# brownvc/gftorf

Measured on AMD Instinct MI355X. Metric: train iters/sec (fwd+bwd raster) + Mpix/s, 1M Gaussians @ 640x480 ToF, higher is better.
Workload: dtype f32; 1 GPU; 1M Gaussians, 640x480, SH deg 3, RGB+ToF phasor, forward+backward; P=1000000, W=640, H=480, sh_degree=3, P_visible=954168, num_rendered=3638471, longest_tile_list=0

## Files before the change

gftorf_amd/_lib.py:

```python
import ctypes as C
import os

_HERE = os.path.dirname(os.path.abspath(__file__))
LIB_PATH = os.path.join(_HERE, "libgftorf_rast.so")
ABI_VERSION = 15
DEFORM_MAX_INPUTS = 96
ACC_STRIDE = 16

_lib = None

_fp = C.c_void_p


class Config(C.Structure):
    _fields_ = [
        ("P", C.c_int32), ("D", C.c_int32), ("M", C.c_int32), ("M_p", C.c_int32),
        ("W", C.c_int32), ("H", C.c_int32),
        ("tanfovx", C.c_float), ("tanfovy", C.c_float), ("scale_modifier", C.c_float),
        ("near_n", C.c_float), ("far_n", C.c_float), ("depth_range", C.c_float),
        ("phase_offset", C.c_float), ("dc_offset", C.c_float),
        ("use_view_dependent_phase", C.c_int32), ("prefiltered", C.c_int32), ("debug", C.c_int32),
        ("want_backward", C.c_int32),
        ("acc_zeroed", C.c_int32),
        ("grads_zeroed", C.c_int32),
# ... 89 lines not shown

class DeformParams(C.Structure):
    _fields_ = [("linear_w", _fp * 8), ("linear_b", _fp * 8), ("xyz_w", _fp), ("xyz_b", _fp), ("r_w", _fp), ("r_b", _fp),
                ("g_w", _fp), ("g_b", _fp), ("b_w", _fp), ("b_b", _fp)]


DEFORM_FIELDS = [f[0] for f in DeformParams._fields_]


class AdamTensor(C.Structure):
    _fields_ = [("param", _fp), ("grad", _fp), ("exp_avg", _fp), ("exp_avg_sq", _fp), ("n", C.c_int64), ("lr", C.c_double),
                ("step", C.c_int64)]

EXPORTS = [
    "gft_abi_version", "gft_lazy_sort", "gft_last_error", "gft_geom_bytes", "gft_image_bytes", "gft_cell_sched_words", "gft_binning_bytes", "gft_acc_bytes",
    "gft_det_partials_bytes", "gft_get_layout", "gft_binning_capacity", "gft_set_binning_mode", "gft_binning_mode", "gft_set_render_mode", "gft_forward_preprocess", "gft_forward_render", "gft_forward", "gft_forward_enqueue", "gft_backward", "gft_grads_rezero",
    "gft_mark_visible", "gft_profile_enable", "gft_profile_reset", "gft_profile_read",
    "gft_assemble_scratch_bytes", "gft_assemble_forward", "gft_assemble_num_dynamic", "gft_assemble_backward",
    "gft_knn_scratch_bytes", "gft_knn_mean_dist2", "gft_adam_step", "gft_adam_step_multi", "gft_adam_step_rows", "gft_adam_step_multi_dev",
    "gft_deform_inputs", "gft_deform_packed_bytes", "gft_deform_saved_bytes", "gft_deform_scratch_bytes", "gft_deform_pack",
    "gft_deform_forward", "gft_deform_backward", "gft_deform_compact", "gft_deform_rows_work_bytes", "gft_deform_backward_rows",
    "gft_ssim_blocks", "gft_ssim_l2_forward", "gft_ssim_l2_backward",
    "gft_image_loss_forward", "gft_image_loss_backward", "gft_pixel_loss_blocks", "gft_pixel_loss_forward", "gft_pixel_loss_backward",
    "gft_densify_stats", "gft_rows_rank_scratch_bytes", "gft_rows_rank", "gft_rows_rank_dev", "gft_rows_gather", "gft_rows_any_nonzero",
]
FLOW_EXPORTS = ["gft_flow_loss_blocks", "gft_flow_loss_forward", "gft_flow_loss_backward", "gft_flow_points", "gft_flow_project",
                "gft_flow_project_backward"]
FEATURE_EXPORTS = ["gft_render_features", "gft_render_features_backward"]


def load():
# ... 16 lines not shown
    lib.gft_image_bytes.argtypes = [C.c_int32, C.c_int32]
    lib.gft_cell_sched_words.restype = C.c_size_t
    lib.gft_cell_sched_words.argtypes = [C.c_int32, C.c_int32]
    lib.gft_binning_bytes.restype = C.c_size_t
    lib.gft_binning_bytes.argtypes = [C.c_int64, C.c_int32, C.c_int32]
    lib.gft_acc_bytes.restype = C.c_size_t
    lib.gft_acc_bytes.argtypes = [C.c_int32]
    lib.gft_det_partials_bytes.restype = C.c_size_t
    lib.gft_det_partials_bytes.argtypes = [C.c_int64, C.c_int32, C.c_int32]
    lib.gft_binning_capacity.restype = C.c_int64
    lib.gft_binning_capacity.argtypes = [C.c_size_t, C.c_int32, C.c_int32]
    lib.gft_set_binning_mode.restype = C.c_int
    lib.gft_set_binning_mode.argtypes = [C.c_int]
    lib.gft_set_render_mode.restype = C.c_int
    lib.gft_set_render_mode.argtypes = [C.c_int]
    lib.gft_binning_mode.restype = C.c_int
    lib.gft_binning_mode.argtypes = [C.POINTER(Config)]
    lib.gft_get_layout.restype = C.c_int
    lib.gft_get_layout.argtypes = [C.c_int32, C.c_int32, C.c_int32, C.c_int64, C.POINTER(Layout)]
    lib.gft_forward_preprocess.restype = C.c_int
    lib.gft_forward_preprocess.argtypes = [C.c_void_p, C.POINTER(Config), C.POINTER(ForwardIO),
                                           C.POINTER(C.c_int64), C.POINTER(C.c_int64)]
    lib.gft_forward_render.restype = C.c_int
    lib.gft_adam_step.restype = C.c_int
    lib.gft_adam_step.argtypes = [C.c_void_p, C.c_int64, C.c_void_p, C.c_void_p, C.c_void_p, C.c_void_p,
                                  C.c_double, C.c_double, C.c_double, C.c_double, C.c_double, C.c_int64]
    lib.gft_adam_step_multi.restype = C.c_int
    lib.gft_adam_step_multi.argtypes = [C.c_void_p, C.c_int32, C.POINTER(AdamTensor), C.c_double, C.c_double, C.c_double,
                                        C.c_double]
    lib.gft_adam_step_multi_dev.restype = C.c_int
# ... 173 lines not shown
```

gftorf_amd/csrc/gft_api.hip:

```cpp
#include "gft_internal.h"

#include <stdarg.h>
#include <stdio.h>
#include <string.h>
#include <cstdlib>
#include <mutex>
#include <vector>

static thread_local char g_err[512] = "";

int gft_fail(const char* fmt, ...)
{
    va_list ap;
    va_start(ap, fmt);
    vsnprintf(g_err, sizeof(g_err), fmt, ap);
    va_end(ap);
    return 1;
}

extern "C" const char* gft_last_error(void) { return g_err; }
extern "C" int gft_abi_version(void) { return GFT_ABI_VERSION; }
static size_t point_list_slots(int64_t binning_instances, int32_t W, int32_t H)
{
    if (binning_instances <= 0) return 0;
// ... 29 lines not shown
    L->geom_need = o;     o = align_up(o + p);
    L->geom_blockhist = o; o = align_up(o + ((p + BIN_CHUNK - 1) / BIN_CHUNK) * GFT_BLOCKHIST_TILES * 2);
    L->geom_total = o;

    const size_t n = (size_t)W * (size_t)H;
    const size_t T = (size_t)((W + GFT_TILE_X - 1) / GFT_TILE_X) * (size_t)((H + GFT_TILE_Y - 1) / GFT_TILE_Y);
    o = 0;
    L->img_pix_state = o;   o = align_up(o + n * 16);
    L->img_ranges = o;      o = align_up(o + T * 8);
    L->img_tile_max = o;    o = align_up(o + T * 4 * 4);
    L->img_ctrl = o;        o += (GFT_CTRL_WORDS + GFT_TICKET_WORDS) * 4;
    L->img_tile_cnt = o;    o += T * 4;
    L->img_tile_cut = o;    o += T * 4;
    L->img_super_tab = o;   o = align_up(o + 4 * (size_t)GFT_SUPER_CELLS * 4);
    L->img_tile_cursor = o; o = align_up(o + T * 4);
    L->img_tile_order = o;  o = align_up(o + T * 4);
    L->img_front_len = o;   o = align_up(o + T * 4);
    L->img_unit_flag = o;   o = align_up(o + T * 16);
    L->img_resume_state = o; o = align_up(o + n * 64);
    L->img_pix_sums = o;    o = align_up(o + n * 32);
    L->img_snaps = o;       o = align_up(o + 4 * T * (size_t)(gft_bwd_segments(T) - 1) * GFT_SNAP_F4 * 64 * 16);
    L->img_total = o;

    const size_t r = (size_t)(R > 0 ? R : 0);
    o = 0;
    L->bin_keys = o;        o = align_up(o + r * 8);
    L->bin_point_list = o;  o = align_up(o + (r ? T * (size_t)GFT_HEAD_SLOT + r : 0) * 4);
    L->bin_total = o + GFT_ALIGN;
}

GeomView gft_geom_view(void* base, const gft_layout& L)
// ... 13 lines not shown
}

ImgView gft_img_view(void* base, const gft_layout& L)
{
    char* b = (char*)base;
    ImgView v;
    v.pix_state = (float4*)(b + L.img_pix_state);
    v.ranges = (uint2*)(b + L.img_ranges);
    v.tile_max = (uint32_t*)(b + L.img_tile_max);
    v.ctrl = (uint32_t*)(b + L.img_ctrl);
    v.tile_cnt = (uint32_t*)(b + L.img_tile_cnt);
    v.tile_cut = (uint32_t*)(b + L.img_tile_cut);
    v.super_tab = (uint32_t*)(b + L.img_super_tab);
    v.tile_cursor = (uint32_t*)(b + L.img_tile_cursor);
    v.tile_order = (uint32_t*)(b + L.img_tile_order);
    v.front_len = (uint32_t*)(b + L.img_front_len);
    v.unit_flag = (uint32_t*)(b + L.img_unit_flag);
    v.resume_state = (float4*)(b + L.img_resume_state);
    v.pix_sums = (float4*)(b + L.img_pix_sums);
    v.snaps = (float4*)(b + L.img_snaps);
    return v;
}

BinView gft_bin_view(void* base, const gft_layout& L)
{
    char* b = (char*)base;
    BinView v;
    v.keys = (uint64_t*)(b + L.bin_keys);
    v.point_list = (uint32_t*)(b + L.bin_point_list);
    return v;
// ... 294 lines not shown
    if (m < 0) {
        const char* e = getenv("GFT_LAZY_BIN");
        m = e ? (atoi(e) != 0) : 1;
        g_binning_mode.store(m);
    }
    return m != 0 && lazy_sort_enabled() && gft_tile_pull_ok(*cfg);
}
extern "C" int gft_binning_mode(const gft_config* cfg) { return (cfg && pull_enabled(cfg)) ? 1 : 0; }

static std::atomic<int> g_render_mode{-2};
extern "C" int gft_set_render_mode(int mode)
{
    g_render_mode.store(mode < 0 ? -2 : (mode ? 1 : 0));
    return 0;
}
int gft_render_mode()
{
    int m = g_render_mode.load();
    if (m == -2) {
        const char* e = getenv("GFT_FWD_SEG");
        m = e ? (atoi(e) != 0 ? 1 : 0) : -1;
        g_render_mode.store(m);
    }
    return m;
}

static int enqueue_count(hipStream_t s, const gft_config* cfg, const gft_forward_io* io, const GeomView& g, const ImgView& im,
                         uint32_t* mail_dev, uint32_t seq, bool pull, int64_t status_cap = -1);

static int enqueue_stage1(hipStream_t s, const gft_config* cfg, const gft_forward_io* io, const GeomView& g,
// ... 131 lines not shown
    if (binning_instances < 0 || binning_instances > 0xffffffffll) return gft_fail("gft_forward_render: bad instance count");
    if (binning_instances > 0 && !io->binning) return gft_fail("gft_forward_render: binning buffer is NULL");
    if (cfg->P > 0 && (!io->geom || !io->radii || !io->pixels)) return gft_fail("gft_forward_render: geom/radii/pixels NULL");
    hipStream_t s = (hipStream_t)hip_stream;
    const int64_t R = cfg->P == 0 ? 0 : binning_instances;
    gft_layout L;
    gft_compute_layout(cfg->P, cfg->W, cfg->H, R, &L);
    GeomView g = gft_geom_view(io->geom, L);
    ImgView im = gft_img_view(io->img, L);
    BinView b = gft_bin_view(io->binning, L);
    const bool pull = cfg->P > 0 && pull_enabled(cfg);
    if (cfg->P == 0 || (pull && R == 0)) {
        const int gx = (cfg->W + GFT_TILE_X - 1) / GFT_TILE_X, gy = (cfg->H + GFT_TILE_Y - 1) / GFT_TILE_Y;
        GFT_CHECK_HIP(gft_zero_async(im.ranges, (size_t)gx * gy * sizeof(uint2), s));
        if (cfg->P == 0) GFT_CHECK_HIP(gft_zero_async(im.ctrl, GFT_CTRL_WORDS * sizeof(uint32_t), s));
    }
    return enqueue_stage2(s, cfg, io, g, im, b, R > 0, max_tile_list, cfg->P > 0, (uint32_t)R, pull, io->tile_hints != nullptr);
}

extern "C" int gft_forward(void* hip_stream, const gft_config* cfg, const gft_forward_io* io,
                           const gft_forward_hints* hints, gft_forward_report* report)
{
    if (report) memset(report, 0, sizeof(*report));
    if (check_config(cfg)) return 1;
    if (!io || !hints || !report) return gft_fail("gft_forward: NULL argument");
    if (check_stage2(io, "gft_forward")) return 1;
    const int64_t binning_instances = hints->binning_instances;
    if (binning_instances < 0 || binning_instances > 0xffffffffll) return gft_fail("gft_forward: bad instance count");
    if (cfg->P == 0) return gft_forward_render(hip_stream, cfg, io, 0, 0);
    if (check_stage1(cfg, io, "gft_forward")) return 1;
// ... 170 lines not shown
```

gftorf_amd/csrc/gft_appearance.h:

```cpp
#pragma once
#include "gft_internal.h"

#pragma clang fp contract(off)

struct PreFwdArgs {
    gft_config c;
    gft_forward_io io;
    GeomView g;
    uint32_t* ctrl;
    uint32_t clear_words;
    uint32_t* mail;
    int defer_appearance;
    float focal_x, focal_y, dist2phase;
    int gx, gy;
    int stage_sh, stage_shp;
    const uint32_t* prev_w;
    uint32_t* fwd_order;
    int T;
};

inline PreFwdArgs gft_pre_fwd_args(const gft_config& c, const gft_forward_io& io, const GeomView& g, const ImgView& im,
                                   uint32_t* mail, bool defer_appearance)
{
    PreFwdArgs a;
    a.c = c;
    a.io = io;
    a.g = g;
    a.ctrl = im.ctrl;
    a.mail = mail;
    a.defer_appearance = defer_appearance ? 1 : 0;
    {
        const size_t T = (size_t)((c.W + GFT_TILE_X - 1) / GFT_TILE_X) * (size_t)((c.H + GFT_TILE_Y - 1) / GFT_TILE_Y);
        a.clear_words = (uint32_t)(GFT_CTRL_WORDS + GFT_TICKET_WORDS + 2 * T + GFT_SUPER_CELLS);
    }
    a.focal_y = c.H / (2.0f * c.tanfovy);
    a.focal_x = c.W / (2.0f * c.tanfovx);
    a.dist2phase = 4.0f * 3.14159265358979323846f / c.depth_range;
    a.gx = (c.W + GFT_TILE_X - 1) / GFT_TILE_X;
    a.gy = (c.H + GFT_TILE_Y - 1) / GFT_TILE_Y;
    a.stage_sh = a.stage_shp = 0;
    a.prev_w = nullptr; a.fwd_order = nullptr; a.T = a.gx * a.gy;
    return a;
}
// ... 347 lines not shown
```

gftorf_amd/csrc/gft_internal.h:

```cpp
#pragma once
#include <hip/hip_runtime.h>
#include <stdint.h>
#include <stddef.h>
#include "gftorf_rast.h"

#include <atomic>
#include <cstdlib>

#define GFT_ALIGN 256

inline hipError_t gft_lds_opt_in(const void* kernel, size_t bytes, std::atomic<uint64_t>& done)
{
    int dev = 0;
    hipError_t e = hipGetDevice(&dev);
    if (e != hipSuccess) return e;
    const uint64_t bit = dev >= 0 && dev < 64 ? 1ull << dev : 0ull;
    if (bit && (done.load(std::memory_order_acquire) & bit)) return hipSuccess;
    e = hipFuncSetAttribute(kernel, hipFuncAttributeMaxDynamicSharedMemorySize, (int)bytes);
    if (e == hipSuccess && bit) done.fetch_or(bit, std::memory_order_release);
    return e;
}
#define GFT_BLOCK 256
#define GFT_NUM_ACC 15

// ... 9 lines not shown
    uint16_t* blockhist;
};

struct ImgView {
    float4* pix_state;
    float4* pix_sums;
    float4* snaps;
    uint2* ranges;
    uint32_t* tile_max;
    uint32_t* ctrl;
    uint32_t* tile_cnt;
    uint32_t* tile_cut;
    uint32_t* super_tab;
    uint32_t* tile_cursor;
    uint32_t* tile_order;
    uint32_t* front_len;
    uint32_t* unit_flag;
    float4* resume_state;
};

struct BinView {
    uint64_t* keys;
    uint32_t* point_list;
};

#define GFT_CTRL_TOTAL 0
#define GFT_CTRL_FLAGS 1
#define GFT_CTRL_MAXCNT 2
#define GFT_CTRL_NFLAG 4
#define GFT_CTRL_DONE 3
// ... 4 lines not shown
#define GFT_CTRL_NHINT 8
#define GFT_CTRL_RSUM 9
#define GFT_CTRL_FWDORDER 10
#define GFT_CTRL_ORDER_OK 11
#define GFT_CTRL_WORDS 16
__device__ __forceinline__ void gft_status_sticky(uint32_t* mail, uint32_t post, uint32_t R)
{
    if (!post) return;
    mail[GFT_STATUS_CAP] = post - 1u;
    if (R > post - 1u) {
        __hip_atomic_fetch_add(&mail[GFT_STATUS_OVERFLOWS], 1u, __ATOMIC_RELAXED, __HIP_MEMORY_SCOPE_SYSTEM);
        __hip_atomic_fetch_max(&mail[GFT_STATUS_MAX_R], R, __ATOMIC_RELAXED, __HIP_MEMORY_SCOPE_SYSTEM);
    }
}
#define GFT_TICKET_WORDS 32
#define GFT_SUPER_MAX 1024
#define GFT_SLAB_MAX 16
#define GFT_SUPER_CELLS (GFT_SUPER_MAX * GFT_SLAB_MAX)
#define GFT_DEPTH_BINS 4096
#define GFT_HEAD_SLOT 2048u
#define GFT_HEAD_DIRECT 2048u
#define GFT_HEAD_TARGET 940u
#define GFT_NO_TAIL 0xffffffffu
#define GFT_BLOCKHIST_TILES 2048
#ifndef BIN_THREADS
#define BIN_THREADS 1024
#endif
#ifndef BIN_ITEMS
#define BIN_ITEMS 4
#endif
// ... 249 lines not shown
```

gftorf_amd/csrc/gft_render_walk.h:

```cpp
#pragma once
#include "gft_internal.h"

struct RenderFwdArgs {
    int W, H, gx, T;
    const uint2* __restrict__ ranges;
    const uint32_t* __restrict__ point_list;
    const float4* __restrict__ rec_a;
    const float4* __restrict__ rec_b;
    const float* __restrict__ bg;
    int64_t bsc, bsy, bsx;
    float dc_offset;
    const float* dc_offset_dev;
    float4* __restrict__ pix_state;
    float4* __restrict__ pix_sums;
    uint32_t* __restrict__ quad_max;
    float* out_color; float* out_phasor; float* out_depth; float* out_normal; float* out_acc;
    float* out_entropy; float* out_dd; float* out_ad; float* out_distribution;
    float* pixels;
    const uint32_t* __restrict__ ctrl;
    uint32_t cap;
    const uint32_t* __restrict__ tile_cut;
    float4* __restrict__ snaps;
    int nsnap;
    const uint32_t* __restrict__ front_len;
    uint32_t* __restrict__ unit_flag;
    uint32_t* nflag;
    float4* __restrict__ resume_state;
    int resume;
    uint8_t* __restrict__ hint_out;
    const uint32_t* __restrict__ fwd_order;
    const uint32_t* __restrict__ fwd_order_ok;
    uint32_t* __restrict__ weights_out;
};

RenderFwdArgs gft_render_fwd_args(const gft_config& c, const gft_forward_io& io, const GeomView& g, const ImgView& im,
                                  const BinView& b, bool check_cap, uint32_t cap, int lazy, bool pull);

namespace {

#define RB 64

__device__ __forceinline__ float gft_exp(float x) { return __builtin_amdgcn_exp2f(x * 1.4426950408889634f); }

__device__ __forceinline__ unsigned long long wave_ballot(bool p) { return __builtin_amdgcn_ballot_w64(p); }

__device__ __forceinline__ float sel_mask(unsigned long long m, float a, float b)
{
// ... 235 lines not shown
```

gftorf_amd/csrc/k_preprocess.hip:

```cpp
#include "gft_internal.h"
#include "gft_appearance.h"
#include <mutex>

#pragma clang fp contract(off)

namespace {

template <int NC>
__device__ __forceinline__ void sh_backward(int deg, int M, float x, float y, float z, const float* sh,
                                            const float* dres, float* dsh, float* ddir)
{
    float ddx[NC], ddy[NC], ddz[NC];
#pragma unroll
    for (int c = 0; c < NC; c++) {
        ddx[c] = 0.f; ddy[c] = 0.f; ddz[c] = 0.f;
        dsh[c] = SH_C0 * dres[c];
    }
    int written = 1;
    if (deg > 0) {
        const float d1 = -SH_C1 * y, d2 = SH_C1 * z, d3 = -SH_C1 * x;
#pragma unroll
        for (int c = 0; c < NC; c++) {
            const float s1 = sh[1 * NC + c], s2 = sh[2 * NC + c], s3 = sh[3 * NC + c];
            ddx[c] = -SH_C1 * s3;
// ... 234 lines not shown
                    store_rec_a(a, idx, sg, vx, vy, vz);
                    if (!a.defer_appearance) appearance_fwd(a, idx, lane, sh_l, shp_l, px, py, pz, vx, vy, vz, phase_offset);
                    radius = (int)sg.my_radius;
                    tiles = area;
                    rect = make_ushort4((unsigned short)x0, (unsigned short)y0, (unsigned short)x1, (unsigned short)y1);
                }
            }
        }
        a.io.radii[idx] = radius;
        a.io.pixels[idx] = 0.0f;
        a.g.tiles[idx] = tiles;
        a.g.rect[idx] = rect;
        a.g.need[idx] = 0;
    }
    for (uint32_t w = (uint32_t)idx; w < a.clear_words; w += gridDim.x * PRE_BLOCK) a.ctrl[w] = 0u;
}

#define APP_THREADS 256
#define APP_CHUNK_OF(words) ((words) * 4 * APP_THREADS)
template <int WORDS>
__global__ __launch_bounds__(APP_THREADS) void k_appearance(PreFwdArgs a, uint32_t cap)
{
    constexpr int APP_CHUNK = APP_CHUNK_OF(WORDS);
    __shared__ uint32_t s_ids[APP_CHUNK];
    __shared__ uint32_t s_n;
    if (a.ctrl[GFT_CTRL_TOTAL] > cap) return;
    const float phase_offset = gft_offset_value(a.io.phase_offset_dev, a.c.phase_offset);
    const int tid = threadIdx.x, lane = tid & 63;
    if (blockIdx.x == 0 && a.prev_w != nullptr && a.prev_w[4 * a.T] == 1u) {
        gft_tile_order_block(a.T, a.prev_w, a.fwd_order);
// ... 722 lines not shown
```

gftorf_amd/csrc/k_render.hip:

```cpp
#include "gft_internal.h"
#include "gft_render_walk.h"

namespace {

typedef unsigned int u32x2 __attribute__((ext_vector_type(2)));

__device__ __forceinline__ int unit_of_block(int b, int V)
{
    const int chunk = (V + 7) >> 3;
    return (b & 7) * chunk + (b >> 3);
}

__global__ __launch_bounds__(64) void k_render_fwd(RenderFwdArgs a)
{
    __shared__ float4 sA[RB * 2];
    __shared__ float4 sB[RB * 2];

    const float dc_offset = gft_offset_value(a.dc_offset_dev, a.dc_offset);
    if (a.ctrl && a.ctrl[GFT_CTRL_TOTAL] > a.cap) return;
    if (a.resume && *a.nflag == 0u) return;
    const int V = a.T * 4;
    int v;
    if (a.fwd_order && *a.fwd_order_ok) {
        const int xcd = (int)blockIdx.x & 7, qslot = (int)blockIdx.x >> 3;
        const int rank = 8 * (qslot >> 2) + xcd;
        if (rank >= a.T) return;
        v = (int)a.fwd_order[rank] * 4 + (qslot & 3);
    } else {
        if (((int)blockIdx.x >> 3) >= ((V + 7) >> 3)) return;
        v = unit_of_block(blockIdx.x, V);
    }
    if (v >= V) return;
    render_fwd_walk(a, v, (int)threadIdx.x, sA, sB, dc_offset);
}

#define FSEG_WAVES_MAX 8
#define FSEG_MIN_LEN 128
#define FSEG_SPEC_MAX 512

template <int FSEG_WAVES>
__global__ __launch_bounds__(64 * FSEG_WAVES) __attribute__((amdgpu_waves_per_eu(7, 7))) void k_render_fwd_seg(RenderFwdArgs a)
{
    __shared__ float4 sStage[FSEG_WAVES][RB * 4];
    __shared__ float sT[FSEG_WAVES][64];
    __shared__ uint8_t sCnt[FSEG_WAVES][FSEG_SPEC_MAX];

    const float dc_offset = gft_offset_value(a.dc_offset_dev, a.dc_offset);
    if (a.ctrl && a.ctrl[GFT_CTRL_TOTAL] > a.cap) return;
// ... 401 lines not shown
    int split;
    int nseg;
    const float4* __restrict__ snaps;
    const uint32_t* __restrict__ front_len;
    const uint32_t* __restrict__ quad_max;
    const uint32_t* __restrict__ order;
    const uint32_t* __restrict__ order_ok;
    const uint32_t* __restrict__ order_fwd;
    const uint32_t* __restrict__ order_fwd_ok;
    const float* __restrict__ g_color; const float* __restrict__ g_phasor; const float* __restrict__ g_depth;
    const float* __restrict__ g_acc; const float* __restrict__ g_dd;
    const uint32_t* __restrict__ ctrl;
    uint32_t cap;
    float* acc;
    float* det;
};

__device__ __forceinline__ float swap32_add(float x, float y)
{
    const u32x2 r = __builtin_amdgcn_permlane32_swap(__float_as_uint(x), __float_as_uint(y), false, false);
    return __uint_as_float(r.x) + __uint_as_float(r.y);
}

__device__ __forceinline__ float swap16_add(float x, float y)
{
    const u32x2 r = __builtin_amdgcn_permlane16_swap(__float_as_uint(x), __float_as_uint(y), false, false);
    return __uint_as_float(r.x) + __uint_as_float(r.y);
}

__device__ __forceinline__ float row_fold4(float t0, float t1, float t2, float t3)
// ... 39 lines not shown

__device__ __forceinline__ float wave_reduce16(v2f L01, v2f L23, v2f L45, v2f L67, v2f H01, v2f H23, v2f H45, v2f H67)
{
    const v2f s01 = swap32_add2(L01, H01), s23 = swap32_add2(L23, H23);
    const v2f s45 = swap32_add2(L45, H45), s67 = swap32_add2(L67, H67);
    const v2f t01 = swap16_add2(s01, s45), t23 = swap16_add2(s23, s67);
    return row_fold4(t01.x, t01.y, t23.x, t23.y);
}

__global__ __launch_bounds__(1024) void k_tile_order(int T, const uint32_t* __restrict__ quad_max,
                                                     uint32_t* __restrict__ order)
{
    gft_tile_order_block(T, quad_max, order);
}

__global__ __launch_bounds__(64) void k_render_bwd(RenderBwdArgs a)
{
    __shared__ float4 sA[RB * 2];
    __shared__ float4 sB[RB * 2];
    __shared__ uint32_t sId[RB];

    if (a.ctrl[GFT_CTRL_TOTAL] > a.cap) return;
    const float dc_offset = gft_offset_value(a.dc_offset_dev, a.dc_offset);
    const int per_seg = (int)gridDim.x / a.nseg;
    const int sgroup = (int)blockIdx.x / per_seg;
    const int bid = (int)blockIdx.x - sgroup * per_seg;
    const int xcd = bid & 7, qslot = bid >> 3;
    const int rank = 8 * (qslot >> 2) + xcd;
    if (rank >= a.T) return;
    const uint32_t* order = a.order;
    bool ordered = order && (a.order_ok == nullptr || *a.order_ok != 0u);
    if (order && a.order_fwd && *a.order_fwd_ok != 0u) { order = a.order_fwd; ordered = true; }
    const int v_unit = (int)(ordered ? order[rank] : (uint32_t)rank) * 4 + (qslot & 3);
    const int tmax = (int)a.quad_max[v_unit];
    if (tmax == 0) return;
    int ncut = 0;
    if (a.split) {
        const int head = a.front_len ? (int)a.front_len[v_unit >> 2] : tmax;
        const int lim = min(tmax, head);
        ncut = lim > 0 ? (lim - 1) / GFT_SEG_LEN : 0;
        if (ncut > a.nseg - 1) ncut = a.nseg - 1;
    }
    const bool front_first = a.T > GFT_FWD_ORDER_MAX_TILES && ncut >= 1 && tmax - ncut * GFT_SEG_LEN <= GFT_SEG_LEN;
    int seg;
    if (sgroup == 0) seg = front_first ? 0 : ncut;
    else if (sgroup == 1) { if (ncut < 1) return; seg = front_first ? ncut : 0; }
    else { seg = sgroup - 1; if (seg >= ncut) return; }
    const int lo_last = seg * GFT_SEG_LEN;
    const int hi_first = seg == ncut ? tmax : lo_last + GFT_SEG_LEN;
    const int tile = v_unit >> 2, quad = v_unit & 3;
    const int lane = threadIdx.x;
    const int tx = tile % a.gx, ty = tile / a.gx;
    const int qx0 = tx * GFT_TILE_X + (quad & 1) * 8, qy0 = ty * GFT_TILE_Y + (quad >> 1) * 8;
    const int px = qx0 + (lane & 7), py = qy0 + (lane >> 3);
    const bool inside = px < a.W && py < a.H;
    const float pxf = (float)px, pyf = (float)py;
    const uint32_t r0 = a.ranges[tile].x;
    auto phys = [&](uint32_t c) -> uint32_t { return r0 + c; };
    const float zref = a.rec_a[2 * a.point_list[phys(0u)] + 1].z;
    const size_t HW = (size_t)a.H * a.W;
    const size_t pix = inside ? (size_t)a.W * py + px : 0;

    float T_final = 0.f, wz_tot = 0.f, wz2_tot = 0.f;
    int n_contrib = 0;
    float gc0 = 0, gc1 = 0, gc2 = 0, gp0 = 0, gp1 = 0, gp2 = 0, gp3 = 0, gp4 = 0, gp5 = 0, gp6 = 0;
    float gd = 0, ga = 0, gdd = 0;
// ... 131 lines not shown
                if (more1) { j1 = (int)__builtin_ctzll(m); m &= m - 1; }
                const float4 r0 = sA[2 * j1], r1 = sA[2 * j1 + 1], t0 = sB[2 * j1], t1 = sB[2 * j1 + 1];
                const uint32_t g1 = sId[j1];
                entry(j0, g0, p0, p1, q0, q1);
                if (!more1) break;
                const bool more0 = m != 0;
                j0 = j1;
                if (more0) { j0 = (int)__builtin_ctzll(m); m &= m - 1; }
                p0 = sA[2 * j0]; p1 = sA[2 * j0 + 1]; q0 = sB[2 * j0]; q1 = sB[2 * j0 + 1];
                g0 = sId[j0];
                entry(j1, g1, r0, r1, t0, t1);
                if (!more0) break;
            }
        }
    }
}

__global__ __launch_bounds__(1024) void k_acc_reduce_det(int T, const uint2* __restrict__ ranges,
                                                         const uint32_t* __restrict__ quad_max,
                                                         const uint32_t* __restrict__ point_list,
                                                         const float* __restrict__ det, float* acc,
                                                         const uint32_t* __restrict__ ctrl, uint32_t cap)
{
    if (ctrl[GFT_CTRL_TOTAL] > cap) return;
    const int tid = threadIdx.x;
    for (int tile = 0; tile < T; tile++) {
        const uint4 qm = reinterpret_cast<const uint4*>(quad_max)[tile];
        const uint32_t walked = max(max(qm.x, qm.y), max(qm.z, qm.w));
        const uint2 rg = ranges[tile];
        for (uint32_t i = (uint32_t)tid; i < walked * GFT_ACC_STRIDE; i += 1024u) {
// ... 40 lines not shown
    a.pix_state = im.pix_state; a.quad_max = im.tile_max;
    a.pix_sums = im.pix_sums;
    a.out_color = io.out_color; a.out_phasor = io.out_phasor; a.out_depth = io.out_depth;
    a.out_normal = io.out_normal; a.out_acc = io.out_acc; a.out_entropy = io.out_entropy;
    a.out_dd = io.out_depth_distortion; a.out_ad = io.out_amp_distortion;
    a.out_distribution = io.out_distribution; a.pixels = io.pixels;
    a.front_len = lazy ? im.front_len : nullptr;
    a.unit_flag = im.unit_flag;
    a.nflag = im.ctrl + GFT_CTRL_NFLAG;
    a.resume_state = im.resume_state;
    a.resume = lazy == 2;
    const bool ordered = pull && lazy == 1 && io.tile_weights != nullptr && gft_fwd_ordered(a.T);
    a.fwd_order = ordered ? im.tile_cursor : nullptr;
    a.fwd_order_ok = im.ctrl + GFT_CTRL_FWDORDER;
    a.weights_out = (pull && lazy != 0 && gft_fwd_ordered(a.T)) ? io.tile_weights : nullptr;
    return a;
}

hipError_t gft_launch_render_fwd(hipStream_t s, const gft_config& c, const gft_forward_io& io, const GeomView& g,
                                 const ImgView& im, const BinView& b, bool check_cap, uint32_t cap, int lazy, bool pull,
                                 bool segmented)
{
    const RenderFwdArgs a = gft_render_fwd_args(c, io, g, im, b, check_cap, cap, lazy, pull);
    const bool ordered = a.fwd_order != nullptr;
    const int blocks = ordered ? 32 * ((a.T + 7) / 8) : 8 * ((a.T * 4 + 7) / 8);
    const bool seg = segmented && !a.resume && gft_fwd_segmented(a.T);
    if (seg) {
        switch (gft_fwd_seg_waves(a.T)) {
        case 2: hipLaunchKernelGGL(k_render_fwd_seg<2>, dim3(blocks), dim3(64 * 2), 0, s, a); break;
        case 3: hipLaunchKernelGGL(k_render_fwd_seg<3>, dim3(blocks), dim3(64 * 3), 0, s, a); break;
        case 4: hipLaunchKernelGGL(k_render_fwd_seg<4>, dim3(blocks), dim3(64 * 4), 0, s, a); break;
        case 5: hipLaunchKernelGGL(k_render_fwd_seg<5>, dim3(blocks), dim3(64 * 5), 0, s, a); break;
        case 6: hipLaunchKernelGGL(k_render_fwd_seg<6>, dim3(blocks), dim3(64 * 6), 0, s, a); break;
        case 7: hipLaunchKernelGGL(k_render_fwd_seg<7>, dim3(blocks), dim3(64 * 7), 0, s, a); break;
        default: hipLaunchKernelGGL(k_render_fwd_seg<8>, dim3(blocks), dim3(64 * 8), 0, s, a); break;
        }
    }
    else hipLaunchKernelGGL(k_render_fwd, dim3(blocks), dim3(64), 0, s, a);
    return hipGetLastError();
}

hipError_t gft_launch_render_bwd(hipStream_t s, const gft_config& c, const gft_backward_io& io, const GeomView& g,
                                 const ImgView& im, const BinView& b, bool lazy, uint32_t cap)
{
    RenderBwdArgs a;
    a.ctrl = im.ctrl; a.cap = cap;
    a.W = c.W; a.H = c.H;
    a.gx = (c.W + GFT_TILE_X - 1) / GFT_TILE_X;
    const int gy = (c.H + GFT_TILE_Y - 1) / GFT_TILE_Y;
    a.T = a.gx * gy;
    a.ranges = im.ranges; a.point_list = b.point_list; a.rec_a = g.rec_a; a.rec_b = g.rec_b;
    a.bg = io.bg; a.bsc = c.bg_stride_c; a.bsy = c.bg_stride_y; a.bsx = c.bg_stride_x;
    a.dc_offset = c.dc_offset; a.dc_offset_dev = io.dc_offset_dev;
// ... 3 lines not shown
    a.acc = io.acc;
    a.det = io.det_partials;
    static const int order_on = [] { const char* e = getenv("GFT_BWD_ORDER"); return e ? atoi(e) != 0 : 1; }();
    a.order = order_on ? im.tile_order : nullptr;
    a.order_ok = lazy ? im.ctrl + GFT_CTRL_ORDER_OK : nullptr;
    a.order_fwd = lazy ? im.tile_cursor : nullptr;
    a.order_fwd_ok = im.ctrl + GFT_CTRL_FWDORDER;
    if (order_on && !lazy) hipLaunchKernelGGL(k_tile_order, dim3(1), dim3(1024), 0, s, a.T, im.tile_max, im.tile_order);
    a.pix_sums = im.pix_sums;
    static const int split_on = [] { const char* e = getenv("GFT_BWD_SPLIT"); return e ? atoi(e) != 0 : 1; }();
    a.nseg = gft_bwd_segments((size_t)a.T);
    a.split = split_on && a.nseg > 1 && c.want_backward;
    if (!a.split) a.nseg = 1;
    a.snaps = im.snaps;
    a.front_len = lazy ? im.front_len : nullptr;
    const int blocks = a.nseg * 32 * ((a.T + 7) / 8);
    hipLaunchKernelGGL(k_render_bwd, dim3(blocks), dim3(64), 0, s, a);
    if (a.det)
        hipLaunchKernelGGL(k_acc_reduce_det, dim3(1), dim3(1024), 0, s, a.T, im.ranges, im.tile_max, b.point_list,
                           a.det, io.acc, im.ctrl, cap);
    return hipGetLastError();
}
```

include/gftorf_rast.h:

```cpp
#ifndef GFTORF_RAST_H
#define GFTORF_RAST_H

#include <stddef.h>
#include <stdint.h>

#ifdef __cplusplus
extern "C" {
#endif

#define GFT_ABI_VERSION 15

#define GFT_NUM_CHANNELS 3
#define GFT_NUM_CHANNELS_PHASOR 7
#define GFT_NUM_CHANNELS_CWTOF 2
#define GFT_TILE_X 16
#define GFT_TILE_Y 16
#define GFT_ACC_STRIDE 16

typedef struct gft_config {
    int32_t P;
    int32_t D;
    int32_t M;
    int32_t M_p;
    int32_t W, H;
// ... 130 lines not shown

int gft_abi_version(void);
int gft_lazy_sort(void);
const char* gft_last_error(void);

size_t gft_geom_bytes(int32_t P);
size_t gft_image_bytes(int32_t W, int32_t H);
size_t gft_cell_sched_words(int32_t W, int32_t H);
size_t gft_binning_bytes(int64_t R, int32_t W, int32_t H);
size_t gft_acc_bytes(int32_t P);
size_t gft_det_partials_bytes(int64_t binning_instances, int32_t W, int32_t H);
int64_t gft_binning_capacity(size_t bytes, int32_t W, int32_t H);
int gft_set_binning_mode(int mode);
int gft_binning_mode(const gft_config* cfg);
int gft_set_render_mode(int mode);
int gft_get_layout(int32_t P, int32_t W, int32_t H, int64_t R, gft_layout* out );

int gft_forward_preprocess(void* hip_stream, const gft_config* cfg,
                           const gft_forward_io* io, int64_t* num_rendered ,
                           int64_t* max_tile_list );

int gft_forward_render(void* hip_stream, const gft_config* cfg,
                       const gft_forward_io* io, int64_t binning_instances,
                       int64_t max_tile_list );

typedef struct gft_forward_hints {
    int64_t binning_instances;
    int64_t max_tile_list;
    int64_t whole_lists;
    int64_t use_cell_sched;
// ... 39 lines not shown
```

Before: 2633 it/s.

## Use persistent per-XCD work queues for forward and backward blend kernels

New measurement: 850.0 it/s. -67.7%, worse.

```diff
diff --git a/gftorf_amd/_lib.py b/gftorf_amd/_lib.py
--- a/gftorf_amd/_lib.py
+++ b/gftorf_amd/_lib.py
@@ -127,7 +127,7 @@
 
 EXPORTS = [
     "gft_abi_version", "gft_lazy_sort", "gft_last_error", "gft_geom_bytes", "gft_image_bytes", "gft_cell_sched_words", "gft_binning_bytes", "gft_acc_bytes",
-    "gft_det_partials_bytes", "gft_get_layout", "gft_binning_capacity", "gft_set_binning_mode", "gft_binning_mode", "gft_set_render_mode", "gft_forward_preprocess", "gft_forward_render", "gft_forward", "gft_forward_enqueue", "gft_backward", "gft_grads_rezero",
+    "gft_det_partials_bytes", "gft_get_layout", "gft_binning_capacity", "gft_set_binning_mode", "gft_binning_mode", "gft_set_render_mode", "gft_set_blend_dispatch", "gft_forward_preprocess", "gft_forward_render", "gft_forward", "gft_forward_enqueue", "gft_backward", "gft_grads_rezero",
     "gft_mark_visible", "gft_profile_enable", "gft_profile_reset", "gft_profile_read",
     "gft_assemble_scratch_bytes", "gft_assemble_forward", "gft_assemble_num_dynamic", "gft_assemble_backward",
     "gft_knn_scratch_bytes", "gft_knn_mean_dist2", "gft_adam_step", "gft_adam_step_multi", "gft_adam_step_rows", "gft_adam_step_multi_dev",
@@ -174,6 +174,8 @@
     lib.gft_set_binning_mode.argtypes = [C.c_int]
     lib.gft_set_render_mode.restype = C.c_int
     lib.gft_set_render_mode.argtypes = [C.c_int]
+    lib.gft_set_blend_dispatch.restype = C.c_int
+    lib.gft_set_blend_dispatch.argtypes = [C.c_int]
     lib.gft_binning_mode.restype = C.c_int
     lib.gft_binning_mode.argtypes = [C.POINTER(Config)]
     lib.gft_get_layout.restype = C.c_int
diff --git a/gftorf_amd/csrc/gft_api.hip b/gftorf_amd/csrc/gft_api.hip
--- a/gftorf_amd/csrc/gft_api.hip
+++ b/gftorf_amd/csrc/gft_api.hip
@@ -67,7 +67,7 @@
     L->img_tile_cut = o;    o += T * 4;
     L->img_super_tab = o;   o = align_up(o + 4 * (size_t)GFT_SUPER_CELLS * 4);
     L->img_tile_cursor = o; o = align_up(o + T * 4);
-    L->img_tile_order = o;  o = align_up(o + T * 4);
+    L->img_tile_order = o;  o = align_up(o + T * 4 + GFT_QUEUE_WORDS * 4);
     L->img_front_len = o;   o = align_up(o + T * 4);
     L->img_unit_flag = o;   o = align_up(o + T * 16);
     L->img_resume_state = o; o = align_up(o + n * 64);
@@ -111,6 +111,7 @@
     v.super_tab = (uint32_t*)(b + L.img_super_tab);
     v.tile_cursor = (uint32_t*)(b + L.img_tile_cursor);
     v.tile_order = (uint32_t*)(b + L.img_tile_order);
+    v.queue = (uint32_t*)(b + L.img_front_len) - GFT_QUEUE_WORDS;
     v.front_len = (uint32_t*)(b + L.img_front_len);
     v.unit_flag = (uint32_t*)(b + L.img_unit_flag);
     v.resume_state = (float4*)(b + L.img_resume_state);
@@ -435,6 +436,23 @@
     g_render_mode.store(mode < 0 ? -2 : (mode ? 1 : 0));
     return 0;
 }
+static std::atomic<int> g_blend_dispatch{-1};
+extern "C" int gft_set_blend_dispatch(int mode)
+{
+    g_blend_dispatch.store(mode < 0 ? -1 : (mode > 4096 ? 4096 : mode));
+    return 0;
+}
+int gft_blend_queue()
+{
+    int m = g_blend_dispatch.load();
+    if (m < 0) {
+        const char* e = getenv("GFT_BLEND_QUEUE");
+        m = e ? (atoi(e) > 0 ? (atoi(e) > 4096 ? 4096 : atoi(e)) : 0) : 1;
+        g_blend_dispatch.store(m);
+    }
+    return m;
+}
+
 int gft_render_mode()
 {
     int m = g_render_mode.load();
@@ -596,6 +614,7 @@
         const int gx = (cfg->W + GFT_TILE_X - 1) / GFT_TILE_X, gy = (cfg->H + GFT_TILE_Y - 1) / GFT_TILE_Y;
         GFT_CHECK_HIP(gft_zero_async(im.ranges, (size_t)gx * gy * sizeof(uint2), s));
         if (cfg->P == 0) GFT_CHECK_HIP(gft_zero_async(im.ctrl, GFT_CTRL_WORDS * sizeof(uint32_t), s));
+        if (cfg->P == 0) GFT_CHECK_HIP(gft_zero_async(im.queue, GFT_QUEUE_WORDS * sizeof(uint32_t), s));
     }
     return enqueue_stage2(s, cfg, io, g, im, b, R > 0, max_tile_list, cfg->P > 0, (uint32_t)R, pull, io->tile_hints != nullptr);
 }
diff --git a/gftorf_amd/csrc/gft_appearance.h b/gftorf_amd/csrc/gft_appearance.h
--- a/gftorf_amd/csrc/gft_appearance.h
+++ b/gftorf_amd/csrc/gft_appearance.h
@@ -9,6 +9,7 @@
     GeomView g;
     uint32_t* ctrl;
     uint32_t clear_words;
+    uint32_t* queue;
     uint32_t* mail;
     int defer_appearance;
     float focal_x, focal_y, dist2phase;
@@ -27,6 +28,7 @@
     a.io = io;
     a.g = g;
     a.ctrl = im.ctrl;
+    a.queue = im.queue;
     a.mail = mail;
     a.defer_appearance = defer_appearance ? 1 : 0;
     {
diff --git a/gftorf_amd/csrc/gft_internal.h b/gftorf_amd/csrc/gft_internal.h
--- a/gftorf_amd/csrc/gft_internal.h
+++ b/gftorf_amd/csrc/gft_internal.h
@@ -47,6 +47,7 @@
     uint32_t* super_tab;
     uint32_t* tile_cursor;
     uint32_t* tile_order;
+    uint32_t* queue;
     uint32_t* front_len;
     uint32_t* unit_flag;
     float4* resume_state;
@@ -81,6 +82,20 @@
     }
 }
 #define GFT_TICKET_WORDS 32
+#define GFT_QUEUE_WORDS 32
+#define GFT_QUEUE_FWD 0
+#define GFT_QUEUE_BWD 16
+#define GFT_QUEUE_EXIT 8
+int gft_blend_queue();
+inline int gft_blend_grid(bool bwd, int units)
+{
+    static const int f = [] { const char* e = getenv("GFT_BLEND_WAVES_FWD"); const int v = e ? atoi(e) : 0; return v > 0 ? (v > 8 ? 8 : v) : 3; }();
+    static const int b = [] { const char* e = getenv("GFT_BLEND_WAVES_BWD"); const int v = e ? atoi(e) : 0; return v > 0 ? (v > 8 ? 8 : v) : 5; }();
+    const int m = gft_blend_queue();
+    if (m == 0) return 0;
+    const int grid = m > 1 ? 8 * m : 1024 * (bwd ? b : f);
+    return units > grid ? grid : 0;
+}
 #define GFT_SUPER_MAX 1024
 #define GFT_SLAB_MAX 16
 #define GFT_SUPER_CELLS (GFT_SUPER_MAX * GFT_SLAB_MAX)
diff --git a/gftorf_amd/csrc/gft_render_walk.h b/gftorf_amd/csrc/gft_render_walk.h
--- a/gftorf_amd/csrc/gft_render_walk.h
+++ b/gftorf_amd/csrc/gft_render_walk.h
@@ -31,6 +31,8 @@
     const uint32_t* __restrict__ fwd_order;
     const uint32_t* __restrict__ fwd_order_ok;
     uint32_t* __restrict__ weights_out;
+    uint32_t* queue;
+    int nslot;
 };
 
 RenderFwdArgs gft_render_fwd_args(const gft_config& c, const gft_forward_io& io, const GeomView& g, const ImgView& im,
diff --git a/gftorf_amd/csrc/k_preprocess.hip b/gftorf_amd/csrc/k_preprocess.hip
--- a/gftorf_amd/csrc/k_preprocess.hip
+++ b/gftorf_amd/csrc/k_preprocess.hip
@@ -272,6 +272,7 @@
         a.g.need[idx] = 0;
     }
     for (uint32_t w = (uint32_t)idx; w < a.clear_words; w += gridDim.x * PRE_BLOCK) a.ctrl[w] = 0u;
+    if (idx < GFT_QUEUE_WORDS) a.queue[idx] = 0u;
 }
 
 #define APP_THREADS 256
diff --git a/gftorf_amd/csrc/k_render.hip b/gftorf_amd/csrc/k_render.hip
--- a/gftorf_amd/csrc/k_render.hip
+++ b/gftorf_amd/csrc/k_render.hip
@@ -9,6 +9,21 @@
 {
     const int chunk = (V + 7) >> 3;
     return (b & 7) * chunk + (b >> 3);
+}
+
+__device__ __forceinline__ void queue_leave(uint32_t* q, int lane)
+{
+    if (lane != 0) return;
+    if (atomicAdd(&q[GFT_QUEUE_EXIT], 1u) != gridDim.x - 1u) return;
+#pragma unroll
+    for (int i = 0; i <= GFT_QUEUE_EXIT; i++) __hip_atomic_store(&q[i], 0u, __ATOMIC_RELAXED, __HIP_MEMORY_SCOPE_AGENT);
+}
+
+__device__ __forceinline__ int queue_pull(uint32_t* cursor, int lane)
+{
+    uint32_t t = 0;
+    if (lane == 0) t = atomicAdd(cursor, 1u);
+    return (int)(gridDim.x >> 3) + (int)__builtin_amdgcn_readfirstlane(t);
 }
 
 __global__ __launch_bounds__(64) void k_render_fwd(RenderFwdArgs a)
@@ -20,18 +35,27 @@
     if (a.ctrl && a.ctrl[GFT_CTRL_TOTAL] > a.cap) return;
     if (a.resume && *a.nflag == 0u) return;
     const int V = a.T * 4;
-    int v;
-    if (a.fwd_order && *a.fwd_order_ok) {
-        const int xcd = (int)blockIdx.x & 7, qslot = (int)blockIdx.x >> 3;
-        const int rank = 8 * (qslot >> 2) + xcd;
-        if (rank >= a.T) return;
-        v = (int)a.fwd_order[rank] * 4 + (qslot & 3);
-    } else {
-        if (((int)blockIdx.x >> 3) >= ((V + 7) >> 3)) return;
-        v = unit_of_block(blockIdx.x, V);
-    }
-    if (v >= V) return;
-    render_fwd_walk(a, v, (int)threadIdx.x, sA, sB, dc_offset);
+    const bool ordered = a.fwd_order && *a.fwd_order_ok;
+    const int xcd = (int)blockIdx.x & 7;
+    auto unit_of_slot = [&](int qslot) -> int {
+        int v;
+        if (ordered) {
+            const int rank = 8 * (qslot >> 2) + xcd;
+            if (rank >= a.T) return -1;
+            v = (int)a.fwd_order[rank] * 4 + (qslot & 3);
+        } else {
+            if (qslot >= ((V + 7) >> 3)) return -1;
+            v = unit_of_block(qslot * 8 + xcd, V);
+        }
+        return v < V ? v : -1;
+    };
+    const int nslot = a.queue ? a.nslot : (int)(gridDim.x >> 3);
+    for (int slot = (int)blockIdx.x >> 3; slot < nslot; slot = queue_pull(&a.queue[xcd], (int)threadIdx.x)) {
+        const int v = unit_of_slot(slot);
+        if (v >= 0) render_fwd_walk(a, v, (int)threadIdx.x, sA, sB, dc_offset);
+        if (a.queue == nullptr) return;
+    }
+    queue_leave(a.queue, (int)threadIdx.x);
 }
 
 #define FSEG_WAVES_MAX 8
@@ -463,6 +487,7 @@
     uint32_t cap;
     float* acc;
     float* det;
+    uint32_t* queue;
 };
 
 __device__ __forceinline__ float swap32_add(float x, float y)
@@ -532,7 +557,7 @@
     gft_tile_order_block(T, quad_max, order);
 }
 
-__global__ __launch_bounds__(64) void k_render_bwd(RenderBwdArgs a)
+__global__ __launch_bounds__(64) __attribute__((amdgpu_waves_per_eu(5, 5))) void k_render_bwd(RenderBwdArgs a)
 {
     __shared__ float4 sA[RB * 2];
     __shared__ float4 sB[RB * 2];
@@ -540,34 +565,40 @@
 
     if (a.ctrl[GFT_CTRL_TOTAL] > a.cap) return;
     const float dc_offset = gft_offset_value(a.dc_offset_dev, a.dc_offset);
-    const int per_seg = (int)gridDim.x / a.nseg;
-    const int sgroup = (int)blockIdx.x / per_seg;
-    const int bid = (int)blockIdx.x - sgroup * per_seg;
-    const int xcd = bid & 7, qslot = bid >> 3;
-    const int rank = 8 * (qslot >> 2) + xcd;
-    if (rank >= a.T) return;
+    const int lane = threadIdx.x;
+    const int xcd = (int)blockIdx.x & 7;
+    const int Q = 4 * ((a.T + 7) / 8), N = a.nseg * Q;
     const uint32_t* order = a.order;
     bool ordered = order && (a.order_ok == nullptr || *a.order_ok != 0u);
     if (order && a.order_fwd && *a.order_fwd_ok != 0u) { order = a.order_fwd; ordered = true; }
-    const int v_unit = (int)(ordered ? order[rank] : (uint32_t)rank) * 4 + (qslot & 3);
-    const int tmax = (int)a.quad_max[v_unit];
-    if (tmax == 0) return;
-    int ncut = 0;
-    if (a.split) {
-        const int head = a.front_len ? (int)a.front_len[v_unit >> 2] : tmax;
-        const int lim = min(tmax, head);
-        ncut = lim > 0 ? (lim - 1) / GFT_SEG_LEN : 0;
-        if (ncut > a.nseg - 1) ncut = a.nseg - 1;
-    }
-    const bool front_first = a.T > GFT_FWD_ORDER_MAX_TILES && ncut >= 1 && tmax - ncut * GFT_SEG_LEN <= GFT_SEG_LEN;
-    int seg;
-    if (sgroup == 0) seg = front_first ? 0 : ncut;
-    else if (sgroup == 1) { if (ncut < 1) return; seg = front_first ? ncut : 0; }
-    else { seg = sgroup - 1; if (seg >= ncut) return; }
+    auto candidate = [&](const int cc, int& v_unit, int& tmax, int& pack) -> bool {
+        const int sgroup = cc / Q;
+        const int qslot = cc - sgroup * Q;
+        const int rank = 8 * (qslot >> 2) + xcd;
+        const bool ok = cc < N && rank < a.T;
+        const int tile = ok ? (int)(ordered ? order[rank] : (uint32_t)rank) : 0;
+        v_unit = tile * 4 + (qslot & 3);
+        tmax = ok ? (int)a.quad_max[v_unit] : 0;
+        int ncut = 0;
+        if (a.split) {
+            const int head = a.front_len ? (int)a.front_len[tile] : tmax;
+            const int lim = min(tmax, head);
+            ncut = lim > 0 ? (lim - 1) / GFT_SEG_LEN : 0;
+            if (ncut > a.nseg - 1) ncut = a.nseg - 1;
+        }
+        const bool front_first = a.T > GFT_FWD_ORDER_MAX_TILES && ncut >= 1 && tmax - ncut * GFT_SEG_LEN <= GFT_SEG_LEN;
+        int seg;
+        bool live = tmax != 0;
+        if (sgroup == 0) seg = front_first ? 0 : ncut;
+        else if (sgroup == 1) { live = live && ncut >= 1; seg = front_first ? ncut : 0; }
+        else { seg = sgroup - 1; live = live && seg < ncut; }
+        pack = seg | (ncut << 8);
+        return live;
+    };
+    auto walk_unit = [&](const int v_unit, const int tmax, const int ncut, const int seg) {
     const int lo_last = seg * GFT_SEG_LEN;
     const int hi_first = seg == ncut ? tmax : lo_last + GFT_SEG_LEN;
     const int tile = v_unit >> 2, quad = v_unit & 3;
-    const int lane = threadIdx.x;
     const int tx = tile % a.gx, ty = tile / a.gx;
     const int qx0 = tx * GFT_TILE_X + (quad & 1) * 8, qy0 = ty * GFT_TILE_Y + (quad >> 1) * 8;
     const int px = qx0 + (lane & 7), py = qy0 + (lane >> 3);
@@ -729,6 +760,37 @@
             }
         }
     }
+    };
+
+    const bool pq = a.queue != nullptr;
+    uint32_t* cursor = pq ? a.queue + xcd : nullptr;
+    const int wpx = (int)gridDim.x >> 3;
+    int c = (int)blockIdx.x >> 3, base = 0;
+    bool have = false;
+    int w_unit = 0, w_tmax = 0, w_pack = 0;
+    uint64_t live_m = 0;
+    while (c < N) {
+        if (!have || c >= base + 64) {
+            base = c;
+            live_m = to_sgpr(wave_ballot(candidate(base + (pq ? lane : 0), w_unit, w_tmax, w_pack)));
+            have = true;
+        }
+        const int j = c - base;
+        const bool live = (live_m >> j) & 1ull;
+        if (pq) {
+            const uint64_t behind = j < 63 ? live_m >> (j + 1) : 0ull;
+            const int skip = behind ? (int)__builtin_ctzll(behind) : 63 - j;
+            if (skip > 0 && c + 1 + skip > wpx && lane == 0) atomicMax(cursor, (uint32_t)(c + 1 + skip - wpx));
+        }
+        if (live) {
+            const int pack = __builtin_amdgcn_readlane(w_pack, j);
+            walk_unit(__builtin_amdgcn_readlane(w_unit, j), __builtin_amdgcn_readlane(w_tmax, j), pack >> 8, pack & 0xff);
+            have = false;
+        }
+        if (!pq) return;
+        c = queue_pull(cursor, lane);
+    }
+    if (pq) queue_leave(a.queue, lane);
 }
 
 __global__ __launch_bounds__(1024) void k_acc_reduce_det(int T, const uint2* __restrict__ ranges,
@@ -799,6 +861,7 @@
     a.fwd_order = ordered ? im.tile_cursor : nullptr;
     a.fwd_order_ok = im.ctrl + GFT_CTRL_FWDORDER;
     a.weights_out = (pull && lazy != 0 && gft_fwd_ordered(a.T)) ? io.tile_weights : nullptr;
+    a.queue = nullptr; a.nslot = 0;
     return a;
 }
 
@@ -806,9 +869,9 @@
                                  const ImgView& im, const BinView& b, bool check_cap, uint32_t cap, int lazy, bool pull,
                                  bool segmented)
 {
-    const RenderFwdArgs a = gft_render_fwd_args(c, io, g, im, b, check_cap, cap, lazy, pull);
+    RenderFwdArgs a = gft_render_fwd_args(c, io, g, im, b, check_cap, cap, lazy, pull);
     const bool ordered = a.fwd_order != nullptr;
-    const int blocks = ordered ? 32 * ((a.T + 7) / 8) : 8 * ((a.T * 4 + 7) / 8);
+    int blocks = ordered ? 32 * ((a.T + 7) / 8) : 8 * ((a.T * 4 + 7) / 8);
     const bool seg = segmented && !a.resume && gft_fwd_segmented(a.T);
     if (seg) {
         switch (gft_fwd_seg_waves(a.T)) {
@@ -821,7 +884,15 @@
         default: hipLaunchKernelGGL(k_render_fwd_seg<8>, dim3(blocks), dim3(64 * 8), 0, s, a); break;
         }
     }
-    else hipLaunchKernelGGL(k_render_fwd, dim3(blocks), dim3(64), 0, s, a);
+    else {
+        const int grid = a.resume ? 0 : gft_blend_grid(false, blocks);
+        if (grid) {
+            a.queue = im.queue + GFT_QUEUE_FWD;
+            a.nslot = blocks / 8;
+            blocks = grid;
+        }
+        hipLaunchKernelGGL(k_render_fwd, dim3(blocks), dim3(64), 0, s, a);
+    }
     return hipGetLastError();
 }
 
@@ -855,7 +926,12 @@
     if (!a.split) a.nseg = 1;
     a.snaps = im.snaps;
     a.front_len = lazy ? im.front_len : nullptr;
-    const int blocks = a.nseg * 32 * ((a.T + 7) / 8);
+    int blocks = a.nseg * 32 * ((a.T + 7) / 8);
+    a.queue = nullptr;
+    if (const int grid = gft_blend_grid(true, blocks)) {
+        a.queue = im.queue + GFT_QUEUE_BWD;
+        blocks = grid;
+    }
     hipLaunchKernelGGL(k_render_bwd, dim3(blocks), dim3(64), 0, s, a);
     if (a.det)
         hipLaunchKernelGGL(k_acc_reduce_det, dim3(1), dim3(1024), 0, s, a.T, im.ranges, im.tile_max, b.point_list,
diff --git a/include/gftorf_rast.h b/include/gftorf_rast.h
--- a/include/gftorf_rast.h
+++ b/include/gftorf_rast.h
@@ -168,6 +168,7 @@
 int gft_set_binning_mode(int mode);
 int gft_binning_mode(const gft_config* cfg);
 int gft_set_render_mode(int mode);
+int gft_set_blend_dispatch(int mode);
 int gft_get_layout(int32_t P, int32_t W, int32_t H, int64_t R, gft_layout* out );
 
 int gft_forward_preprocess(void* hip_stream, const gft_config* cfg,
diff --git a/profiles/experiments/blend_queue_model.c b/profiles/experiments/blend_queue_model.c
--- /dev/null
+++ b/profiles/experiments/blend_queue_model.c
@@ -0,0 +1,44 @@
+#include <math.h>
+#include <stdint.h>
+#include <stddef.h>
+
+#define SEG 256
+
+void gfto_blend_units(int W, int H, int maxseg, const uint32_t* ranges, const uint32_t* point_list, const float* means2D,
+                      const float* conic_opacity, const uint32_t* n_contrib, uint32_t* out_walk, uint32_t* out_hits)
+{
+    const int gx = (W + 15) / 16, gy = (H + 15) / 16;
+#pragma omp parallel for schedule(dynamic, 4)
+    for (int unit = 0; unit < gx * gy * 4; unit++) {
+        const int tile = unit >> 2, quad = unit & 3;
+        const int tx = tile % gx, ty = tile / gx;
+        const int qx0 = tx * 16 + (quad & 1) * 8, qy0 = ty * 16 + (quad >> 1) * 8;
+        const uint32_t r0 = ranges[2 * tile];
+        uint32_t tmax = 0;
+        for (int l = 0; l < 64; l++) {
+            const int px = qx0 + (l & 7), py = qy0 + (l >> 3);
+            if (px < W && py < H && n_contrib[(size_t)W * py + px] > tmax) tmax = n_contrib[(size_t)W * py + px];
+        }
+        out_walk[unit] = tmax;
+        for (int s = 0; s < maxseg; s++) out_hits[(size_t)unit * maxseg + s] = 0;
+        for (uint32_t c = 0; c < tmax; c++) {
+            const uint32_t id = point_list[r0 + c];
+            const float* co = conic_opacity + 4 * (size_t)id;
+            const float mx = means2D[2 * id], my = means2D[2 * id + 1];
+            int hit = 0;
+            for (int l = 0; l < 64 && !hit; l++) {
+                const int px = qx0 + (l & 7), py = qy0 + (l >> 3);
+                if (!(px < W && py < H) || c >= n_contrib[(size_t)W * py + px]) continue;
+                const float dx = mx - (float)px, dy = my - (float)py;
+                const float power = -0.5f * (co[0] * dx * dx + co[2] * dy * dy) - co[1] * dx * dy;
+                if (power > 0.0f) continue;
+                const float alpha = co[3] * expf(power);
+                if ((alpha > 0.99f ? 0.99f : alpha) < 1.0f / 255.0f) continue;
+                hit = 1;
+            }
+            int s = (int)(c / SEG);
+            if (s >= maxseg) s = maxseg - 1;
+            out_hits[(size_t)unit * maxseg + s] += (uint32_t)hit;
+        }
+    }
+}
diff --git a/profiles/experiments/blend_queue_model.py b/profiles/experiments/blend_queue_model.py
--- /dev/null
+++ b/profiles/experiments/blend_queue_model.py
@@ -0,0 +1,147 @@
+import ctypes as C
+import json
+import os
+import subprocess
+import sys
+import tempfile
+
+HERE = os.path.dirname(os.path.abspath(__file__))
+ROOT = os.path.dirname(os.path.dirname(HERE))
+sys.path.insert(0, ROOT)
+sys.path.insert(0, os.path.join(ROOT, "tests"))
+import numpy as np
+from gftorf_amd import synth
+from oracle import oracle
+import helpers as Hh
+
+SEG, MAXSEG, SAT, DEAD = 256, 16, 3.0, 8.0
+HEAD_DIRECT, HEAD_TARGET, ORDER_MAX_TILES = 2048, 940, 4096
+SIMDS = 128
+
+so = os.path.join(tempfile.gettempdir(), "blend_queue_model.so")
+subprocess.check_call(["gcc", "-O2", "-fopenmp", "-fPIC", "-shared", "-o", so, os.path.join(HERE, "blend_queue_model.c"), "-lm"])
+L = C.CDLL(so)
+
+
+def simulate(feed, cap, dead_time):
+    rem = np.full((SIMDS, cap), np.inf)
+    wall = np.full((SIMDS, cap), np.inf)
+    nxt, now, n = 0, 0.0, len(feed)
+
+    def fill(s, j):
+        nonlocal nxt
+        rem[s, j] = wall[s, j] = np.inf
+        while nxt < n:
+            w = feed[nxt]
+            nxt += 1
+            if w > 0:
+                rem[s, j] = w
+                return
+            if dead_time > 0:
+                wall[s, j] = dead_time
+                return
+
+    for j in range(cap):
+        for s in range(SIMDS):
+            fill(s, j)
+    while True:
+        live = np.isfinite(rem)
+        if not live.any() and not np.isfinite(wall).any():
+            return now
+        act = live.sum(1, keepdims=True)
+        rate = np.minimum(1.0 / SAT, 1.0 / np.maximum(act, 1))
+        t_live = np.where(live, rem / rate, np.inf)
+        dt = min(t_live.min(), wall.min())
+        now += dt
+        rem = np.where(live, rem - dt * rate, rem)
+        wall = wall - dt
+        for s, j in zip(*np.nonzero((live & (rem <= 1e-9)) | (wall <= 1e-9))):
+            fill(s, j)
+
+
+def model(name):
+    sc = synth.make_scene(name)
+    f, _ = Hh.run_oracle(oracle, sc, backward=False)
+    g = f.geom
+    W, Hh_ = f.W, f.H
+    gx, gy = (W + 15) // 16, (Hh_ + 15) // 16
+    T = gx * gy
+    p = lambda a: C.c_void_p(a.ctypes.data)
+    arrs = [np.ascontiguousarray(x) for x in (f.ranges, np.asarray(f.point_list, np.uint32), g["means2D"], g["conic_opacity"], f.img["n_contrib"])]
+    walk = np.zeros(4 * T, np.uint32)
+    hits = np.zeros((4 * T, MAXSEG), np.uint32)
+    L.gfto_blend_units(C.c_int(W), C.c_int(Hh_), C.c_int(MAXSEG), *[p(a) for a in arrs], p(walk), p(hits))
+    walk = walk.astype(np.int64)
+    hits = hits.astype(np.float64)
+    full = (np.asarray(f.ranges).reshape(-1, 2)[:, 1] - np.asarray(f.ranges).reshape(-1, 2)[:, 0]).astype(np.int64)
+    head = np.repeat(np.where(full <= HEAD_DIRECT, full, HEAD_TARGET), 4)
+    nseg = max(1, min(8, 65536 // (4 * T)))
+    lim = np.minimum(walk, head)
+    ncut = np.minimum(np.where(lim > 0, (lim - 1) // SEG, 0), nseg - 1)
+    walked_in = np.clip(walk[:, None] - SEG * np.arange(MAXSEG)[None, :], 0, SEG).astype(np.float64)
+    work_seg = hits + walked_in / 8.0
+    wt = walk.reshape(T, 4).max(1)
+    ordered = T <= ORDER_MAX_TILES
+    bucket = 63 - np.minimum(63, (wt * (64.0 / (wt.max() + 1))).astype(np.int64))
+    order = np.argsort(bucket, kind="stable") if ordered else np.arange(T)
+    res = {"tiles": T, "quadrants_with_walk": int((walk > 0).sum()), "mean_walk": float(walk[walk > 0].mean()),
+           "p99_walk": float(np.percentile(walk[walk > 0], 99)), "mean_hits": float(hits.sum(1)[walk > 0].mean()), "nseg": nseg}
+
+    fw = work_seg.sum(1)
+    span = {"a": 0.0}
+    span.update({"b%d" % k: 0.0 for k in range(2, 6)})
+    for x in range(8):
+        if ordered:
+            tiles = order[x::8]
+            feed = fw[(tiles[:, None] * 4 + np.arange(4)[None, :]).ravel()]
+        else:
+            chunk = (4 * T + 7) // 8
+            feed = fw[x * chunk:(x + 1) * chunk]
+        feed = np.maximum(feed, 1e-3)
+        span["a"] = max(span["a"], simulate(feed, int(np.ceil(len(feed) / SIMDS)), 0.0))
+        for k in range(2, 6):
+            span["b%d" % k] = max(span["b%d" % k], simulate(feed, k, 0.0))
+    ideal = fw.sum() / (8 * SIMDS)
+    res["fwd"] = {k: v / ideal for k, v in span.items()}
+
+    last = np.array([work_seg[u, ncut[u]:].sum() for u in range(4 * T)])
+    front_first = (T > ORDER_MAX_TILES) & (ncut >= 1) & (walk - ncut * SEG <= SEG)
+    span = {"a": 0.0}
+    span.update({"b%d" % k: 0.0 for k in range(2, 6)})
+    units = cand = 0
+    total = 0.0
+    for x in range(8):
+        tiles = order[x::8]
+        u = (tiles[:, None] * 4 + np.arange(4)[None, :]).ravel()
+        groups = []
+        g0 = np.where(front_first[u], work_seg[u, 0], last[u]) * (walk[u] > 0)
+        groups.append(g0)
+        if nseg > 1:
+            groups.append(np.where(ncut[u] >= 1, np.where(front_first[u], last[u], work_seg[u, 0]), 0.0))
+        for grp in range(2, nseg):
+            groups.append(np.where(grp - 1 < ncut[u], work_seg[u, grp - 1], 0.0))
+        feed = np.concatenate(groups)
+        feed = np.where(feed > 0, np.maximum(feed, 1e-3), 0.0)
+        units += int((feed > 0).sum())
+        cand += len(feed)
+        total += feed.sum()
+        span["a"] = max(span["a"], simulate(feed, 5, DEAD))
+        for k in range(2, 6):
+            span["b%d" % k] = max(span["b%d" % k], simulate(feed, k, 0.0))
+    ideal = total / (8 * SIMDS)
+    res["bwd"] = {k: v / ideal for k, v in span.items()}
+    res["bwd_workgroups"] = cand
+    res["bwd_workgroups_with_unit"] = units
+    return res
+
+
+out = {}
+for name in ([a for a in sys.argv[1:] if not a.startswith("--")] or ["metric", "C2", "fog", "C5"]):
+    r = out[name] = model(name)
+    print("%s: %d tiles, %d quadrants walk (mean %.0f, p99 %.0f entries, %.0f hits); backward: %d of %d workgroups have a unit (nseg %d)"
+          % (name, r["tiles"], r["quadrants_with_walk"], r["mean_walk"], r["p99_walk"], r["mean_hits"], r["bwd_workgroups_with_unit"],
+             r["bwd_workgroups"], r["nseg"]), flush=True)
+    for kern in ("fwd", "bwd"):
+        print("  %s makespan / ideal: today %.3f | queue " % (kern, r[kern]["a"]) + ", ".join("k=%d %.3f" % (k, r[kern]["b%d" % k]) for k in range(2, 6)), flush=True)
+if "--json" in sys.argv:
+    print(json.dumps(out))
```
